# zypher-game/uzkge

Measured on AMD Instinct MI355X. Metric: bn254_g1_msm_points_per_sec, higher is better.
Workload: dtype u256 (254-bit modular integers: 8 x u32 Montgomery limbs in HBM, 9 x 29-bit limbs in the two hot loops); 1 GPU; BN254 G1 MSM, 2^24 random points + uniform scalars per GPU, bases resident in HBM; points_per_gpu=16777216, total_points=16777216

## Files before the change

uzkge_amd/csrc/fp256.hpp:

```cpp
#pragma once
#include <cstdint>

#if defined(__HIPCC__)
#include <hip/hip_runtime.h>
#define UZK_HD __host__ __device__ __forceinline__
#else
#define UZK_HD inline
#endif

namespace uzk {

struct alignas(16) Fp {
    uint32_t v[8];
};

struct FqCfg {
    static constexpr uint32_t M[8] = {0xd87cfd47u, 0x3c208c16u, 0x6871ca8du, 0x97816a91u,
                                      0x8181585du, 0xb85045b6u, 0xe131a029u, 0x30644e72u};
    static constexpr uint32_t R1[8] = {0xc58f0d9du, 0xd35d438du, 0xf5c70b3du, 0x0a78eb28u,
                                       0x7879462cu, 0x666ea36fu, 0x9a07df2fu, 0x0e0a77c1u};
    static constexpr uint32_t R2[8] = {0x538afa89u, 0xf32cfc5bu, 0xd44501fbu, 0xb5e71911u,
                                       0x0a417ff6u, 0x47ab1effu, 0xcab8351fu, 0x06d89f71u};
    static constexpr uint32_t INV = 0xe4866389u;
    static constexpr uint32_t M2[8] = {0xb0f9fa8eu, 0x7841182du, 0xd0e3951au, 0x2f02d522u,
                                       0x0302b0bbu, 0x70a08b6du, 0xc2634053u, 0x60c89ce5u};
};
struct FrCfg {
    static constexpr uint32_t M[8] = {0xf0000001u, 0x43e1f593u, 0x79b97091u, 0x2833e848u,
                                      0x8181585du, 0xb85045b6u, 0xe131a029u, 0x30644e72u};
    static constexpr uint32_t R1[8] = {0x4ffffffbu, 0xac96341cu, 0x9f60cd29u, 0x36fc7695u,
                                       0x7879462eu, 0x666ea36fu, 0x9a07df2fu, 0x0e0a77c1u};
    static constexpr uint32_t R2[8] = {0xae216da7u, 0x1bb8e645u, 0xe35c59e3u, 0x53fe3ab1u,
                                       0x53bb8085u, 0x8c49833du, 0x7f4e44a5u, 0x0216d0b1u};
    static constexpr uint32_t INV = 0xefffffffu;
    static constexpr uint32_t M2[8] = {0xe0000002u, 0x87c3eb27u, 0xf372e122u, 0x5067d090u,
                                       0x0302b0bau, 0x70a08b6du, 0xc2634053u, 0x60c89ce5u};
};

#if defined(__HIP_DEVICE_COMPILE__)
template <class C>
__device__ __forceinline__ Fp mont_mul_fips(const Fp& a, const Fp& b);
template <class C>
__device__ __forceinline__ Fp fp_add_asm(const Fp& a, const Fp& b);
template <class C>
__device__ __forceinline__ Fp fp_sub_asm(const Fp& a, const Fp& b);
template <class C>
__device__ __forceinline__ Fp mont_mul_fips_relaxed(const Fp& a, const Fp& b);
template <class C>
__device__ __forceinline__ Fp fp_add_2m_asm(const Fp& a, const Fp& b);
template <class C>
__device__ __forceinline__ Fp fp_sub_2m_asm(const Fp& a, const Fp& b);
template <class C>
__device__ __forceinline__ void fp_reduce_once_asm(Fp& r);
#endif

template <class C>
struct Field {
    UZK_HD static Fp zero() { Fp r; for (int i = 0; i < 8; ++i) r.v[i] = 0; return r; }
    UZK_HD static Fp one() { Fp r; for (int i = 0; i < 8; ++i) r.v[i] = C::R1[i]; return r; }
    UZK_HD static Fp modulus() { Fp r; for (int i = 0; i < 8; ++i) r.v[i] = C::M[i]; return r; }
    UZK_HD static bool is_zero(const Fp& a) {
        uint32_t o = 0;
        for (int i = 0; i < 8; ++i) o |= a.v[i];
        return o == 0;
    }
    UZK_HD static bool eq(const Fp& a, const Fp& b) {
        uint32_t o = 0;
        for (int i = 0; i < 8; ++i) o |= a.v[i] ^ b.v[i];
        return o == 0;
    }
    UZK_HD static Fp reduce_once(const Fp& a) {
        Fp d; uint64_t br = 0;
        for (int i = 0; i < 8; ++i) {
            uint64_t t = (uint64_t)a.v[i] - C::M[i] - br;
            d.v[i] = (uint32_t)t; br = (t >> 32) & 1;
        }
        Fp r;
        for (int i = 0; i < 8; ++i) r.v[i] = br ? a.v[i] : d.v[i];
        return r;
    }
    UZK_HD static Fp add(const Fp& a, const Fp& b) {
#if defined(__HIP_DEVICE_COMPILE__) && !defined(UZK_PORTABLE_MUL)
        return fp_add_asm<C>(a, b);
#else
        return add_portable(a, b);
#endif
    }
    UZK_HD static Fp add_portable(const Fp& a, const Fp& b) {
        Fp s; uint64_t c = 0;
        for (int i = 0; i < 8; ++i) { c += (uint64_t)a.v[i] + b.v[i]; s.v[i] = (uint32_t)c; c >>= 32; }
        return reduce_once(s);
    }
    UZK_HD static Fp sub(const Fp& a, const Fp& b) {
#if defined(__HIP_DEVICE_COMPILE__) && !defined(UZK_PORTABLE_MUL)
        return fp_sub_asm<C>(a, b);
#else
        return sub_portable(a, b);
#endif
    }
    UZK_HD static Fp sub_portable(const Fp& a, const Fp& b) {
        Fp d; uint64_t br = 0;
        for (int i = 0; i < 8; ++i) {
            uint64_t t = (uint64_t)a.v[i] - b.v[i] - br;
            d.v[i] = (uint32_t)t; br = (t >> 32) & 1;
        }
        uint32_t mask = (uint32_t)0 - (uint32_t)br;
        uint64_t c = 0;
        for (int i = 0; i < 8; ++i) { c += (uint64_t)d.v[i] + (C::M[i] & mask); d.v[i] = (uint32_t)c; c >>= 32; }
        return d;
    }
    UZK_HD static Fp neg(const Fp& a) {
        Fp d; uint64_t br = 0;
        for (int i = 0; i < 8; ++i) {
            uint64_t t = (uint64_t)C::M[i] - a.v[i] - br;
            d.v[i] = (uint32_t)t; br = (t >> 32) & 1;
        }
        bool z = is_zero(a);
        for (int i = 0; i < 8; ++i) d.v[i] = z ? 0u : d.v[i];
        return d;
    }
    UZK_HD static Fp dbl(const Fp& a) { return add(a, a); }

    UZK_HD static Fp mul(const Fp& a, const Fp& b) {
#if defined(__HIP_DEVICE_COMPILE__) && !defined(UZK_PORTABLE_MUL)
        return mont_mul_fips<C>(a, b);
#else
        return mul_portable(a, b);
#endif
    }
    UZK_HD static Fp mul_portable(const Fp& a, const Fp& b) {
#if !defined(__HIP_DEVICE_COMPILE__)
        return mul_host64(a, b);
#else
        return mul_cios32(a, b);
#endif
    }
#if !defined(__HIP_DEVICE_COMPILE__)
    static inline Fp mul_host64(const Fp& a, const Fp& b) {
        typedef unsigned __int128 u128;
        uint64_t x[4], y[4], m[4];
        for (int i = 0; i < 4; ++i) {
            x[i] = (uint64_t)a.v[2 * i] | ((uint64_t)a.v[2 * i + 1] << 32);
            y[i] = (uint64_t)b.v[2 * i] | ((uint64_t)b.v[2 * i + 1] << 32);
            m[i] = (uint64_t)C::M[2 * i] | ((uint64_t)C::M[2 * i + 1] << 32);
        }
        const uint64_t i32 = C::INV;
        const uint64_t inv = i32 * (2 + m[0] * i32);
        uint64_t t[6] = {0, 0, 0, 0, 0, 0};
        for (int i = 0; i < 4; ++i) {
            u128 c = 0;
            for (int j = 0; j < 4; ++j) { c += (u128)x[j] * y[i] + t[j]; t[j] = (uint64_t)c; c >>= 64; }
            c += t[4]; t[4] = (uint64_t)c; t[5] = (uint64_t)(c >> 64);
            const uint64_t q = t[0] * inv;
            c = (u128)q * m[0] + t[0]; c >>= 64;
            for (int j = 1; j < 4; ++j) { c += (u128)q * m[j] + t[j]; t[j - 1] = (uint64_t)c; c >>= 64; }
            c += t[4]; t[3] = (uint64_t)c; t[4] = t[5] + (uint64_t)(c >> 64);
        }
        Fp r;
        for (int i = 0; i < 4; ++i) { r.v[2 * i] = (uint32_t)t[i]; r.v[2 * i + 1] = (uint32_t)(t[i] >> 32); }
        return reduce_once(r);
    }
#endif
    UZK_HD static Fp mul_cios32(const Fp& a, const Fp& b) {
        uint32_t t[9];
        for (int i = 0; i < 9; ++i) t[i] = 0;
#pragma unroll
        for (int i = 0; i < 8; ++i) {
            uint64_t c = 0;
#pragma unroll
            for (int j = 0; j < 8; ++j) {
                c = (uint64_t)a.v[j] * b.v[i] + t[j] + c;
                t[j] = (uint32_t)c; c >>= 32;
            }
            uint32_t t8 = t[8] + (uint32_t)c;
            uint32_t m = t[0] * C::INV;
            c = (uint64_t)m * C::M[0] + t[0];
            c >>= 32;
#pragma unroll
            for (int j = 1; j < 8; ++j) {
                c = (uint64_t)m * C::M[j] + t[j] + c;
                t[j - 1] = (uint32_t)c; c >>= 32;
            }
            c += t8;
            t[7] = (uint32_t)c; t[8] = (uint32_t)(c >> 32);
        }
        Fp r;
        for (int i = 0; i < 8; ++i) r.v[i] = t[i];
        return reduce_once(r);
    }
    UZK_HD static Fp sqr(const Fp& a) { return mul(a, a); }
#if defined(__HIP_DEVICE_COMPILE__)
    __device__ __forceinline__ static Fp mul_rx(const Fp& a, const Fp& b) { return mont_mul_fips_relaxed<C>(a, b); }
    __device__ __forceinline__ static Fp sub_rx(const Fp& a, const Fp& b) { return fp_sub_2m_asm<C>(a, b); }
    __device__ __forceinline__ static Fp add_rx(const Fp& a, const Fp& b) { return fp_add_2m_asm<C>(a, b); }
    __device__ __forceinline__ static Fp dbl_rx(const Fp& a) { return fp_add_2m_asm<C>(a, a); }
    __device__ __forceinline__ static bool is_zero_rx(const Fp& a) {
        uint32_t z = 0, m = 0;
        for (int i = 0; i < 8; ++i) { z |= a.v[i]; m |= a.v[i] ^ C::M[i]; }
        return z == 0 || m == 0;
    }
    __device__ __forceinline__ static Fp canon(const Fp& a) { Fp r = a; fp_reduce_once_asm<C>(r); return r; }
#elif defined(__HIPCC__)
    __device__ static Fp mul_rx(const Fp& a, const Fp& b);
    __device__ static Fp sub_rx(const Fp& a, const Fp& b);
    __device__ static Fp add_rx(const Fp& a, const Fp& b);
    __device__ static Fp dbl_rx(const Fp& a);
    __device__ static bool is_zero_rx(const Fp& a);
    __device__ static Fp canon(const Fp& a);
#endif
    UZK_HD static Fp from_mont(const Fp& a) {
        Fp o = zero(); o.v[0] = 1;
        return mul(a, o);
    }
    UZK_HD static Fp to_mont(const Fp& a) {
        Fp r2; for (int i = 0; i < 8; ++i) r2.v[i] = C::R2[i];
        return mul(a, r2);
    }
};

using Fq = Field<FqCfg>;
using Fr = Field<FrCfg>;

#if defined(__HIP_DEVICE_COMPILE__)
#include "mont_mul_gfx950.inc"
#endif

}
```

uzkge_amd/csrc/msm.hip:

```cpp
#include <algorithm>
#include <cmath>
#include <mutex>
#include <functional>
#include <memory>
#include <condition_variable>
#include <atomic>
#include <cstring>
#include <thread>
#include <vector>

#include "ctx.hpp"
#include "ec29.hpp"
#include "ecquad.hpp"
#include "ecquad29.hpp"
#include "ec29l.hpp"
#include "host_ec64.hpp"
#include "host_math.hpp"

namespace uzk {

constexpr uint32_t kSeg = 16;
constexpr uint32_t kSignBit = 0x80000000u;
constexpr uint32_t kCombineFan = 32;
constexpr int kMaxPasses = 3;

struct MsmWork {
    DevBuf digits, bucket_count, bucket_start, sorted, buckets, partials, win_sums, class_sums, big;
    DevBuf ent[2];
    DevBuf counts[kMaxPasses], segs_start[kMaxPasses], segs_len[kMaxPasses], items[kMaxPasses];
    DevBuf lvl_cnt[2], lvl_off[2], lvl_part[2], small, task_desc, exc;
    XYZZ* h_sums = nullptr;
    size_t h_sums_cap = 0;
    uint32_t* h_max = nullptr;
};

__host__ __device__ inline int msm_num_windows(int c) {
    int W = (254 + c - 1) / c;
    if (254 - (W - 1) * c == c) ++W;
    return W;
}

__device__ __forceinline__ uint32_t msm_fold_scalar_sign(Fp& k) {
    bool gt = false, decided = false;
#pragma unroll
    for (int j = 7; j >= 0; --j) {
        const uint32_t two_k = (k.v[j] << 1) | (j ? (k.v[j - 1] >> 31) : 0u);
        if (!decided && two_k != FrCfg::M[j]) { gt = two_k > FrCfg::M[j]; decided = true; }
    }
    if (!gt) return 0u;
    k = Fr::neg(k);
    return kSignBit;
}


__global__ __launch_bounds__(256) void msm_digits_kernel(ScalarView scalars, uint32_t* __restrict__ digits,
                                                         uint32_t n, uint32_t batch, int c, int W, int w0, int wcnt,
                                                         uint32_t* __restrict__ zero8 = nullptr) {
    const uint64_t t = (uint64_t)blockIdx.x * blockDim.x + threadIdx.x;
    if (zero8 != nullptr && t < 8) zero8[t] = 0;
    if (t >= (uint64_t)n * batch) return;
    const uint32_t b = (uint32_t)(t / n), i = (uint32_t)(t % n);
    Fp k = Fr::from_mont(scalars.at(b, i));
    const uint32_t flip = msm_fold_scalar_sign(k);
    const uint32_t mask = (1u << c) - 1, half = 1u << (c - 1);
    uint32_t carry = 0;
    uint32_t* dst = digits + (size_t)b * wcnt * n + i;
    for (int w = 0; w < w0 + wcnt && w < W; ++w) {
        uint32_t d = (k.v[0] & mask) + carry;
#pragma unroll
        for (int j = 0; j < 7; ++j) k.v[j] = __funnelshift_r(k.v[j], k.v[j + 1], c);
        k.v[7] >>= c;
        uint32_t out;
        if (d > half) { out = ((1u << c) - d) | kSignBit; carry = 1; }
        else { out = d; carry = 0; }
        if (out & ~kSignBit) out ^= flip;
        if (w >= w0) dst[(size_t)(w - w0) * n] = out;
    }
}

__global__ __launch_bounds__(1024) void msm_digits_hist_kernel(ScalarView scalars, uint32_t* __restrict__ digits,
                                                               uint32_t n, int c, int W, uint32_t shift, uint32_t bins,
                                                               uint32_t* __restrict__ counts) {
    extern __shared__ uint32_t hist[];
    const uint32_t ch = blockIdx.x, nch = gridDim.x, b = blockIdx.y;
    const uint32_t cs = (n + nch - 1) / nch;
    const uint32_t lo = min(n, ch * cs), hi = min(n, lo + cs);
    for (uint32_t k = threadIdx.x; k < (uint32_t)W * bins; k += blockDim.x) hist[k] = 0;
    __syncthreads();
    const uint32_t mask = (1u << c) - 1, half = 1u << (c - 1), bmask = bins - 1;
    for (uint32_t i = lo + threadIdx.x; i < hi; i += blockDim.x) {
        Fp k = Fr::from_mont(scalars.at(b, i));
        const uint32_t flip = msm_fold_scalar_sign(k);
        uint32_t carry = 0;
        uint32_t* dst = digits + (size_t)b * W * n + i;
        for (int w = 0; w < W; ++w) {
            uint32_t d = (k.v[0] & mask) + carry;
#pragma unroll
            for (int j = 0; j < 7; ++j) k.v[j] = __funnelshift_r(k.v[j], k.v[j + 1], c);
            k.v[7] >>= c;
            uint32_t out;
            if (d > half) { out = ((1u << c) - d) | kSignBit; carry = 1; }
            else { out = d; carry = 0; }
            if (out & ~kSignBit) out ^= flip;
            dst[(size_t)w * n] = out;
            const uint32_t mag = out & ~kSignBit;
            if (mag) atomicAdd(&hist[(uint32_t)w * bins + (((mag - 1) >> shift) & bmask)], 1u);
        }
    }
    __syncthreads();
    for (uint32_t k = threadIdx.x; k < (uint32_t)W * bins; k += blockDim.x) {
        const uint32_t w = k / bins, bin = k % bins;
        counts[(((size_t)b * W + w) * nch + ch) * bins + bin] = hist[k];
    }
}

struct RadixArgs {
    const uint32_t* digits;
    const uint2* in_entries;
    const uint32_t* seg_start;
    const uint32_t* seg_len;
    uint32_t n;
    uint32_t remap_cnt;
    uint32_t remap_stride, remap_off;
    const uint32_t* item_off;
    uint32_t nseg, chunk;
    uint32_t shift, mask, bins;
    uint32_t* counts;
    uint32_t* prefix;
    uint32_t* bin_base;
    uint32_t* bin_count;
    uint2* out_entries;
    uint32_t* out_vals;
    uint32_t pk_in_bits, pk_out_bits;
    uint32_t seg_min_len;
};
__device__ __forceinline__ uint32_t pk_key(uint32_t e, uint32_t idx_bits) { return e >> (idx_bits + 1); }
__device__ __forceinline__ uint32_t pk_val(uint32_t e, uint32_t idx_bits) {
    return (e & ((1u << idx_bits) - 1)) | (((e >> idx_bits) & 1u) << 31);
}
__device__ __forceinline__ uint32_t pk_make(uint32_t key_low, uint32_t val, uint32_t idx_bits) {
    return (key_low << (idx_bits + 1)) | ((val >> 31) << idx_bits) | (val & ~kSignBit);
}

template <bool FROM_DIGITS>
__device__ __forceinline__ bool radix_work(const RadixArgs& a, uint32_t item, uint32_t& seg, size_t& cidx, uint32_t& base,
                                           uint32_t& lo, uint32_t& hi) {
    if constexpr (FROM_DIGITS) {
        const uint32_t ch = blockIdx.x, nch = gridDim.x;
        seg = blockIdx.y;
        cidx = ((size_t)seg * nch + ch) * a.bins;
        base = 0;
        const uint32_t cs = (a.n + nch - 1) / nch;
        lo = min(a.n, ch * cs);
        hi = min(a.n, lo + cs);
        return true;
    } else {
        if (item >= a.item_off[a.nseg]) return false;
        uint32_t l = 0, h = a.nseg;
        while (h - l > 1) {
            const uint32_t mid = (l + h) >> 1;
            if (a.item_off[mid] <= item) l = mid; else h = mid;
        }
        seg = l;
        cidx = (size_t)item * a.bins;
        base = a.seg_start[seg];
        const uint32_t len = a.seg_len[seg];
        lo = min(len, (item - a.item_off[seg]) * a.chunk);
        hi = min(len, lo + a.chunk);
        return true;
    }
}
template <bool FROM_DIGITS, bool PK_IN>
__device__ __forceinline__ bool radix_load(const RadixArgs& a, uint32_t seg, uint32_t base, uint32_t k, uint32_t& key,
                                           uint32_t& val) {
    if constexpr (FROM_DIGITS) {
        const uint32_t d = a.digits[(size_t)seg * a.n + k];
        const uint32_t mag = d & ~kSignBit;
        key = mag - 1;
        uint32_t idx = k;
        if (a.remap_cnt) idx = (k / a.remap_cnt) * a.remap_stride + a.remap_off + (k % a.remap_cnt);
        val = idx | (d & kSignBit);
        return mag != 0;
    } else if constexpr (PK_IN) {
        const uint32_t e = reinterpret_cast<const uint32_t*>(a.in_entries)[(size_t)base + k];
        key = pk_key(e, a.pk_in_bits);
        val = pk_val(e, a.pk_in_bits);
        return true;
    } else {
        const uint2 e = a.in_entries[(size_t)base + k];
        key = e.x;
        val = e.y;
        return true;
    }
}

template <bool FROM_DIGITS, bool PK_IN>
__global__ __launch_bounds__(1024) void msm_radix_hist_kernel(RadixArgs a) {
    __shared__ uint32_t cnt[512];
    for (uint32_t item = blockIdx.x;; item += gridDim.x) {
        uint32_t seg, base, lo, hi;
        size_t cidx;
        if (!radix_work<FROM_DIGITS>(a, item, seg, cidx, base, lo, hi)) return;
        for (uint32_t b = threadIdx.x; b < a.bins; b += blockDim.x) cnt[b] = 0;
        __syncthreads();
        for (uint32_t k = lo + threadIdx.x; k < hi; k += blockDim.x) {
            if constexpr (FROM_DIGITS) {
                const uint32_t mag = a.digits[(size_t)seg * a.n + k] & ~kSignBit;
                if (mag) atomicAdd(&cnt[((mag - 1) >> a.shift) & a.mask], 1u);
            } else if constexpr (PK_IN) {
                const uint32_t e = reinterpret_cast<const uint32_t*>(a.in_entries)[(size_t)base + k];
                atomicAdd(&cnt[(pk_key(e, a.pk_in_bits) >> a.shift) & a.mask], 1u);
            } else {
                atomicAdd(&cnt[(a.in_entries[(size_t)base + k].x >> a.shift) & a.mask], 1u);
            }
        }
        __syncthreads();
        uint32_t* dst = a.counts + cidx;
        for (uint32_t b = threadIdx.x; b < a.bins; b += blockDim.x) dst[b] = cnt[b];
        if constexpr (FROM_DIGITS) return;
        __syncthreads();
    }
}

__global__ __launch_bounds__(512) void msm_radix_scan_kernel(RadixArgs a, uint32_t nch, const uint32_t* __restrict__ out_start_of,
                                                             uint32_t out_stride) {
    __shared__ uint32_t wsum[8];
    const uint32_t seg = blockIdx.x, b = threadIdx.x, G = gridDim.y, g = blockIdx.y;
    if (a.seg_min_len && a.seg_len[seg] <= a.seg_min_len) return;
    uint32_t run = 0;
    if (b < a.bins) {
        size_t first = (size_t)seg * nch;
        uint32_t cnt = nch;
        if (a.item_off) { first = a.item_off[seg]; cnt = a.item_off[seg + 1] - a.item_off[seg]; }
        const uint32_t per = (cnt + G - 1) / G;
        const uint32_t c0 = min(cnt, g * per), c1 = min(cnt, c0 + per);
        const uint32_t* p0 = a.counts + first * a.bins + b;
        uint32_t r0 = 0, r1 = 0, r2 = 0, r3 = 0;
        uint32_t ch = 0;
        for (; ch + 4 <= c0; ch += 4) {
            r0 += p0[(size_t)ch * a.bins];
            r1 += p0[(size_t)(ch + 1) * a.bins];
            r2 += p0[(size_t)(ch + 2) * a.bins];
            r3 += p0[(size_t)(ch + 3) * a.bins];
        }
        for (; ch < c0; ++ch) r0 += p0[(size_t)ch * a.bins];
        run = r0 + r1 + r2 + r3;
        for (ch = c0; ch < c1; ++ch) {
            const size_t at = (first + ch) * a.bins + b;
            const uint32_t v = a.counts[at];
            a.prefix[at] = run;
            run += v;
        }
    }
    if (g + 1 != G) return;
    uint32_t incl = run;
    for (int o = 1; o < 64; o <<= 1) {
        const uint32_t t = __shfl_up((int)incl, o);
        if ((int)(b & 63) >= o) incl += t;
    }
    if ((b & 63) == 63) wsum[b >> 6] = incl;
    __syncthreads();
    uint32_t pre = 0;
    for (uint32_t w = 0; w < (b >> 6); ++w) pre += wsum[w];
    const uint32_t excl = pre + incl - run;
    if (b < a.bins) {
        const uint32_t start = out_start_of ? out_start_of[seg] : seg * out_stride;
        a.bin_base[(size_t)seg * a.bins + b] = start + excl;
        a.bin_count[(size_t)seg * a.bins + b] = run;
    }
}

__global__ __launch_bounds__(1024) void msm_radix_items_kernel(const uint32_t* __restrict__ seg_len, uint32_t nseg,
                                                               uint32_t chunk, uint32_t* __restrict__ item_off, uint32_t min_len) {
    __shared__ uint32_t part[1024];
    const uint32_t tid = threadIdx.x;
    const uint32_t per = (nseg + 1023) / 1024;
    const uint32_t lo = min(nseg, tid * per), hi = min(nseg, lo + per);
    uint32_t s = 0;
    auto items_of = [&](uint32_t k) { const uint32_t l = seg_len[k]; return l > min_len ? (l + chunk - 1) / chunk : 0u; };
    for (uint32_t k = lo; k < hi; ++k) s += items_of(k);
    part[tid] = s;
    __syncthreads();
    for (uint32_t off = 1; off < 1024; off <<= 1) {
        uint32_t v = (tid >= off) ? part[tid - off] : 0;
        __syncthreads();
        part[tid] += v;
        __syncthreads();
    }
// ... 1432 lines not shown
        g.class_s = 8;
        g.nb2 = std::max<uint32_t>(256, g.NBL >> 8);
    }
    const uint64_t all_entries = (uint64_t)W_total * n * batch;
    const uint64_t mean_pop = (pre ? (uint64_t)W_total * n : (uint64_t)n) >> g.kb;
    g.L = (uint32_t)std::max<uint64_t>(16, std::min<uint64_t>(256, std::min<uint64_t>(4 * mean_pop, all_entries / 200000)));
    g.bound0 = g.entries / g.L + g.TBK;
    g.part_cap = g.bound0 + 2 * g.TBK;
    g.P = g.kb <= 9 ? 1 : (g.kb <= 18 ? 2 : 3);
    g.pk_bits = 0;
    if (g.P == 2 && (!pre || idx_span)) {
        uint32_t ib = 1;
        while ((1ull << ib) < (pre ? idx_span : (uint64_t)g.seg_n)) ++ib;
        const uint32_t first_bits = std::min<uint32_t>(9, g.kb - 1);
        if (ib + 1 + (g.kb - first_bits) <= 32) g.pk_bits = ib;
    }
    uint32_t rem = g.kb, nseg = g.S0;
    for (int p = 0; p < g.P; ++p) {
        uint32_t bits = (rem + (uint32_t)(g.P - p) - 1) / (uint32_t)(g.P - p);
        if (g.pk_bits && p == 0) bits = std::min<uint32_t>(9, g.kb - 1);
        rem -= bits;
        g.sp[p].shift = rem;
        g.sp[p].bins = 1u << bits;
        g.sp[p].nseg = nseg;
        const uint64_t avg = std::max<uint64_t>(1, (g.S0 * (uint64_t)g.seg_n) / nseg);
        g.sp[p].nch = (uint32_t)std::max<uint64_t>(1, std::min<uint64_t>(1024, avg / 32768));
        if (p == 0 && g.pk_bits && avg <= (1ull << 25)) g.sp[p].nch = (uint32_t)((avg + 32767) / 32768);
        g.sp[p].chunk = (p == g.P - 1) ? 16384u : 32768u;
        g.sp[p].items_bound = (uint32_t)(g.entries / g.sp[p].chunk) + nseg;
        nseg *= g.sp[p].bins;
    }
    MsmWork& m = *g.m;
    UZK_TRY(m.digits.reserve((size_t)g.entries * 4));
    UZK_TRY(m.sorted.reserve((size_t)g.entries * 4));
    UZK_TRY(m.bucket_count.reserve((size_t)g.TBK * 4));
    UZK_TRY(m.bucket_start.reserve((size_t)g.TBK * 4));
    UZK_TRY(m.buckets.reserve((size_t)g.TBK * sizeof(XYZZ)));
    UZK_TRY(m.partials.reserve((size_t)2 * g.RW * std::max<uint32_t>(g.groups, g.class_s ? 2 * (g.nb2 / 256 + 1) : 0) * sizeof(XYZZ)));
    UZK_TRY(m.win_sums.reserve((size_t)g.RW * 2 * sizeof(XYZZ)));
    if (g.class_s) UZK_TRY(m.class_sums.reserve((size_t)g.RW * 2 * g.nb2 * sizeof(XYZZ)));
    for (int p = 0; p < g.P; ++p) {
        UZK_TRY(m.counts[p].reserve((size_t)(p == 0 ? 2 * g.sp[p].nseg * g.sp[p].nch : g.sp[p].items_bound) * g.sp[p].bins * 4));
        if (p > 0) UZK_TRY(m.items[p].reserve(((size_t)g.sp[p].nseg + 1) * 4));
        if (p + 1 < g.P) {
            UZK_TRY(m.segs_start[p].reserve((size_t)g.sp[p].nseg * g.sp[p].bins * 4));
            UZK_TRY(m.segs_len[p].reserve((size_t)g.sp[p].nseg * g.sp[p].bins * 4));
            UZK_TRY(m.ent[p & 1].reserve((size_t)g.entries * sizeof(uint2)));
        }
    }
    for (int k = 0; k < 2; ++k) {
        UZK_TRY(m.lvl_cnt[k].reserve((size_t)g.TBK * 4));
        UZK_TRY(m.lvl_off[k].reserve((size_t)g.TBK * 4));
    }
    UZK_TRY(m.lvl_part[0].reserve((size_t)g.part_cap * sizeof(XYZZ)));
    UZK_TRY(m.small.reserve(16384));
    UZK_TRY(m.task_desc.reserve((size_t)g.bound0 * sizeof(TaskDesc)));
    UZK_TRY(m.exc.reserve((size_t)g.bound0 * 4));
    if (m.h_sums_cap < (size_t)g.RW * 2) {
        if (m.h_sums) (void)hipHostFree(m.h_sums);
        UZK_HIP(hipHostMalloc(reinterpret_cast<void**>(&m.h_sums), (size_t)g.RW * 2 * sizeof(XYZZ), hipHostMallocDefault));
        m.h_sums_cap = (size_t)g.RW * 2;
    }
    if (!m.h_max) UZK_HIP(hipHostMalloc(reinterpret_cast<void**>(&m.h_max), 64, hipHostMallocDefault));
    return UZK_OK;
}

static int msm_group_phase1(Ctx& c, MsmGroup& g, const Affine* points, const ScalarView& d_scalars, uint32_t pre_stride,
                            uint32_t pre_off, bool direct_ok = true) {
    MsmWork& m = *g.m;
    hipStream_t st = g.st;
    c.cur_stream = st;
    uint32_t* digits = m.digits.as<uint32_t>();
    uint32_t* sorted = m.sorted.as<uint32_t>();
    uint32_t* bcount = m.bucket_count.as<uint32_t>();
    uint32_t* bstart = m.bucket_start.as<uint32_t>();
    uint32_t* sm = m.small.as<uint32_t>();
    uint32_t* win_tot = sm;
    uint32_t* d_max = sm + 3200;
    UZK_HIP(hipMemsetAsync(d_max, 0, (3912 - 3200) * 4, st));
    const bool fused_hist = !g.pre && g.w0 == 0 && g.W == g.W_total && g.sp[0].nch >= 256 &&
                            (size_t)g.W * g.sp[0].bins * 4 <= 64 * 1024;
    if (fused_hist) {
        KernelScope ks(c, "msm_digits");
        hipLaunchKernelGGL(msm_digits_hist_kernel, dim3(g.sp[0].nch, g.batch), dim3(1024), (size_t)g.W * g.sp[0].bins * 4, st,
                           d_scalars, digits, g.n32, g.cb, (int)g.W, g.sp[0].shift, g.sp[0].bins, m.counts[0].as<uint32_t>());
    } else {
        KernelScope ks(c, "msm_digits");
        const uint64_t tot = (uint64_t)g.n32 * g.batch;
        hipLaunchKernelGGL(msm_digits_kernel, dim3((unsigned)((tot + 255) / 256)), dim3(256), 0, st, d_scalars, digits, g.n32,
                           g.batch, g.cb, (int)g.W_total, (int)g.w0, (int)g.W, (uint32_t*)nullptr);
    }
    for (int p = 0; p < g.P; ++p) {
        const bool first = (p == 0), last = (p == g.P - 1);
        const SortPass& sp = g.sp[p];
        RadixArgs a{};
        a.shift = sp.shift; a.bins = sp.bins; a.mask = sp.bins - 1;
        a.counts = m.counts[p].as<uint32_t>();
        a.prefix = first ? a.counts + (size_t)sp.nseg * sp.nch * sp.bins : a.counts;
        if (first) {
            a.digits = digits;
            a.n = g.seg_n;
            if (g.pre) { a.remap_cnt = g.n32; a.remap_stride = pre_stride; a.remap_off = pre_off; }
        } else {
            a.in_entries = m.ent[(p - 1) & 1].as<uint2>();
            a.seg_start = m.segs_start[p - 1].as<uint32_t>();
            a.seg_len = m.segs_len[p - 1].as<uint32_t>();
        }
        if (g.pk_bits) { if (first) a.pk_out_bits = g.pk_bits; else a.pk_in_bits = g.pk_bits; }
        if (last) { a.bin_base = bstart; a.bin_count = bcount; a.out_vals = sorted; }
        else {
            a.bin_base = m.segs_start[p].as<uint32_t>(); a.bin_count = m.segs_len[p].as<uint32_t>();
            a.out_entries = m.ent[p & 1].as<uint2>();
        }
        int seg_cfg = -1;
        if (last && !first && g.P == 2 && a.pk_in_bits && c.tune_seg_sort && sp.bins <= 512) {
            const double mean = (double)g.seg_n / (double)g.sp[0].bins;
            const double need = mean + 8.0 * std::sqrt(mean) + 64.0;
            for (int k = 0; k < kSegCfgs; ++k)
                if ((double)kSegCap[k] >= need) { seg_cfg = k; break; }
            if (c.tune_seg_sort >= 10) seg_cfg = std::min(kSegCfgs - 1, c.tune_seg_sort - 10);
            if (seg_cfg >= 0) a.seg_min_len = kSegCap[seg_cfg];
        }
        if (!first) {
            a.item_off = m.items[p].as<uint32_t>();
            a.nseg = sp.nseg;
            a.chunk = sp.chunk;
            KernelScope ks(c, "msm_sort_items");
            hipLaunchKernelGGL(msm_radix_items_kernel, dim3(1), dim3(1024), 0, st, a.seg_len, a.nseg, a.chunk,
                               m.items[p].as<uint32_t>(), a.seg_min_len);
        }
        const dim3 grid = first ? dim3(sp.nch, sp.nseg) : dim3(seg_cfg >= 0 ? std::min<uint32_t>(sp.items_bound, 2048u) : sp.items_bound);
        {
            const size_t wgs = first ? 2 * (size_t)grid.x * grid.y : (size_t)sp.items_bound;
            const size_t ent_bytes = g.pk_bits ? 4 : sizeof(uint2);
            const bool ok = m.counts[p].cap >= wgs * sp.bins * 4 &&
                            (last ? (m.bucket_start.cap >= (size_t)sp.nseg * sp.bins * 4 && m.bucket_count.cap >= (size_t)sp.nseg * sp.bins * 4 &&
                                     m.sorted.cap >= (size_t)g.entries * 4)
                                  : (m.segs_start[p].cap >= (size_t)sp.nseg * sp.bins * 4 && m.segs_len[p].cap >= (size_t)sp.nseg * sp.bins * 4 &&
                                     m.ent[p & 1].cap >= (size_t)g.entries * ent_bytes)) &&
                            (first || m.items[p].cap >= ((size_t)sp.nseg + 1) * 4);
            if (!ok) { set_error("msm: sort pass %d: a workspace is smaller than its launch needs (internal error)", p); return UZK_ERR_DEVICE; }
        }
        if (seg_cfg >= 0) {
            KernelScope ks(c, "msm_sort_segment");
            const dim3 sgrid(sp.nseg);
            switch (seg_cfg) {
                case 0: hipLaunchKernelGGL((msm_radix_segment_kernel<128, 12, 1536>), sgrid, dim3(128), 0, st, a); break;
                case 1: hipLaunchKernelGGL((msm_radix_segment_kernel<256, 12, 3072>), sgrid, dim3(256), 0, st, a); break;
                case 2: hipLaunchKernelGGL((msm_radix_segment_kernel<256, 24, 6144>), sgrid, dim3(256), 0, st, a); break;
                case 3: hipLaunchKernelGGL((msm_radix_segment_kernel<256, 40, 10240>), sgrid, dim3(256), 0, st, a); break;
                case 4: hipLaunchKernelGGL((msm_radix_segment_kernel<512, 40, 18432>), sgrid, dim3(512), 0, st, a); break;
                default: hipLaunchKernelGGL((msm_radix_segment_kernel<512, 72, 18432>), sgrid, dim3(512), 0, st, a); break;
            }
        }
        if (!(first && fused_hist)) {
            KernelScope ks(c, "msm_sort_hist");
            if (first) hipLaunchKernelGGL((msm_radix_hist_kernel<true, false>), grid, dim3(1024), 0, st, a);
            else if (a.pk_in_bits) hipLaunchKernelGGL((msm_radix_hist_kernel<false, true>), grid, dim3(256), 0, st, a);
            else hipLaunchKernelGGL((msm_radix_hist_kernel<false, false>), grid, dim3(256), 0, st, a);
        }
        {
            KernelScope ks(c, "msm_sort_scan");
            const uint32_t scan_g = first ? std::max<uint32_t>(1, std::min<uint32_t>(sp.nch / 16, 1024 / std::max<uint32_t>(1, sp.nseg))) : 1u;
            hipLaunchKernelGGL(msm_radix_scan_kernel, dim3(sp.nseg, scan_g), dim3(512), 0, st, a, sp.nch,
                               first ? (const uint32_t*)nullptr : a.seg_start, first ? g.seg_n : 0u);
        }
        {
            KernelScope ks(c, "msm_sort_scatter");
            const uint32_t cs0 = first ? (g.seg_n + sp.nch - 1) / sp.nch : 0u;
            if (first && !last && a.pk_out_bits && sp.bins <= 512 && cs0 <= 32768 && !g.pre)
                hipLaunchKernelGGL((msm_radix_chunk_kernel<512, 64, 18176>), grid, dim3(512), 0, st, a);
            else if (first && last) hipLaunchKernelGGL((msm_radix_scatter_kernel<1024, 8, true, true, false>), grid, dim3(1024), 0, st, a);
            else if (first && g.entries >= (1ull << 26))
                hipLaunchKernelGGL((msm_radix_scatter_kernel<512, 8, true, false, false>), grid, dim3(512), 0, st, a);
            else if (first) hipLaunchKernelGGL((msm_radix_scatter_kernel<1024, 8, true, false, false>), grid, dim3(1024), 0, st, a);
            else if (last && a.pk_in_bits) hipLaunchKernelGGL((msm_radix_scatter_kernel<512, 8, false, true, true>), grid, dim3(512), 0, st, a);
            else if (last) hipLaunchKernelGGL((msm_radix_scatter_kernel<256, 16, false, true, false>), grid, dim3(256), 0, st, a);
            else hipLaunchKernelGGL((msm_radix_scatter_kernel<1024, 8, false, false, false>), grid, dim3(1024), 0, st, a);
        }
    }
    g.cnt_cur = m.lvl_cnt[0].as<uint32_t>();
    g.off_cur = m.lvl_off[0].as<uint32_t>();
    g.base_cur = sm + 1024;
    g.part_cur = m.lvl_part[0].as<XYZZ>();
    uint32_t* len_hist = sm + 3328;
    uint32_t* len_cur = sm + 3328 + kLenBins;
    g.direct = direct_ok;
    XYZZ* direct_buckets = g.direct ? m.buckets.as<XYZZ>() : nullptr;
    {
        KernelScope ks(c, "msm_scan_win");
        hipLaunchKernelGGL(msm_scan_win_kernel, dim3(g.Wd), dim3(1024), scan_win_lds(g.NB), st, bcount, g.L, g.cnt_cur, g.off_cur, win_tot,
                           d_max, g.NB, len_hist);
        hipLaunchKernelGGL(msm_win_base_kernel, dim3(1), dim3(1024), 0, st, win_tot, g.base_cur, g.Wd);
    }
    TaskDesc* desc = m.task_desc.as<TaskDesc>();
    {
        KernelScope ks(c, "msm_task_order");
        uint32_t* big_count = sm + 3908;
        UZK_TRY(m.big.reserve((size_t)(g.TBK + 1) * sizeof(BigBucket)));
        hipLaunchKernelGGL(msm_task_scan_kernel, dim3(1), dim3(256), 0, st, len_hist, len_cur);
        hipLaunchKernelGGL(msm_bucket_fill_kernel, dim3((unsigned)((g.TBK + 255) / 256)), dim3(256), 0, st, g.base_cur, g.cnt_cur, g.off_cur,
                           bstart, bcount, g.NB, g.TBK, len_cur, desc, big_count, m.big.as<BigBucket>(), g.direct ? 1u : 0u);
        hipLaunchKernelGGL(msm_task_fill_big_kernel, dim3(1024), dim3(64), 0, st, big_count, m.big.as<BigBucket>(), len_cur, desc);
    }
    {
        KernelScope ks(c, "msm_accumulate");
        const dim3 grid((unsigned)((g.bound0 + 255) / 256));
        uint32_t* exc_count = sm + 3900;
        uint32_t* exc_list = m.exc.as<uint32_t>();
        hipLaunchKernelGGL(msm_accumulate29_kernel, grid, dim3(256), 0, st, points, sorted, desc, g.base_cur, g.part_cur,
                           g.Wd, exc_count, exc_list, direct_buckets);
        hipLaunchKernelGGL(msm_accumulate_exc_kernel, dim3(std::min<unsigned>(grid.x, 128u)), dim3(256), 0, st, points, sorted, desc, g.part_cur,
                           exc_count, exc_list, direct_buckets);
    }
    UZK_HIP(hipGetLastError());
    UZK_HIP(hipMemcpyAsync(m.h_max, d_max, 4, hipMemcpyDeviceToHost, st));
    return UZK_OK;
}

static int msm_group_phase2(Ctx& c, MsmGroup& g, bool accumulate = false, bool reduce = true) {
    const int a29 = (c.tune_arith29 >> 2) & 1;
    MsmWork& m = *g.m;
    hipStream_t st = g.st;
    c.cur_stream = st;
    UZK_HIP(hipStreamSynchronize(st));
    uint32_t* sm = m.small.as<uint32_t>();
    uint32_t* win_tot = sm;
    uint32_t* win_base[2] = {sm + 1024, sm + 2080};
    XYZZ* buckets = m.buckets.as<XYZZ>();
    XYZZ* partials = m.partials.as<XYZZ>();
    XYZZ* win_sums = m.win_sums.as<XYZZ>();
    const uint32_t G = kCombineFan;
    uint64_t tmax = ((uint64_t)m.h_max[0] + g.L - 1) / g.L;
    const uint32_t gs = g.TBK >= (1u << 18) ? 1u : (tmax > 2 ? 4u : 1u);
    constexpr uint32_t kBigThresh = 4;
    static_assert(sizeof(BigFold) == sizeof(BigBucket), "the two lists share one buffer");
    const bool big_mode = gs == 1 && tmax > kBigThresh;
    uint32_t* big_count = sm + 3904;
    BigFold* big_list = nullptr;
    if (big_mode) {
        UZK_TRY(m.big.reserve((size_t)(g.bound0 / G + g.TBK + 1) * sizeof(BigFold)));
// ... 203 lines not shown
}
bool msm_small_applies(Ctx& c, size_t n, uint32_t batch, int pre_c = 0) {
    if (!c.tune_small || n == 0 || n > (1u << 15)) return false;
    if (pre_c > 10 || (pre_c == 0 && c.msm_window_bits > 10)) return false;
    const int cb = pre_c > 0 ? pre_c : small_window_bits(c, n, batch);
    const uint64_t S = (uint64_t)batch * (uint64_t)msm_num_windows(cb);
    return S <= 65535 && S * n < (1ull << 31);
}

static int msm_run_small(Ctx& c, const Affine* points, const ScalarView& d_scalars, size_t n, uint32_t batch, Jac* out_host, int pre_c,
                         uint32_t pre_stride, uint32_t pre_off) {
    MsmWork& m = c.msm[0];
    hipStream_t st = c.stream;
    c.cur_stream = st;
    const int cb = pre_c > 0 ? pre_c : small_window_bits(c, n, batch);
    const uint32_t W = (uint32_t)msm_num_windows(cb), S = batch * W, NBL = 1u << (cb - 1), n32 = (uint32_t)n;
    const uint64_t entries = (uint64_t)S * n;
    uint32_t L = 0;
    {
        const double lanes = 0.93 * 64.0 * 4.0 * (double)c.num_cus;
        for (int k = 1; k <= 4; ++k) {
            L = (uint32_t)((double)entries / (lanes * k)) + 1;
            if (L <= 12) break;
        }
        L = std::max<uint32_t>(L, 2);
    }
    const uint64_t task_cap = entries / L + (uint64_t)S * NBL;
    SmallLevels lv{};
    uint64_t cap[kSmallMaxLevels + 1];
    cap[0] = task_cap;
    {
        uint64_t worst = (n + L - 1) / L;
        while (worst > 1 && lv.nl < (uint32_t)kSmallMaxLevels) { worst = (worst + kSmallFan - 1) / kSmallFan; ++lv.nl; }
        if (worst > 1) { set_error("msm: small pipeline: %u fold levels do not cover n = %zu at task length %u", lv.nl, n, L); return UZK_ERR_PARAMETER; }
    }
    uint64_t p_total = 0, d_total = 0;
    for (uint32_t k = 0; k <= lv.nl; ++k) {
        if (k > 0) cap[k] = cap[k - 1] / kSmallFan + (uint64_t)S * NBL;
        lv.pbase[k] = (uint32_t)p_total;
        lv.dbase[k] = (uint32_t)d_total;
        p_total += cap[k];
        if (k > 0) d_total += cap[k];
    }
    if (p_total >= (1ull << 32)) { set_error("msm: small pipeline: too many partial sums"); return UZK_ERR_PARAMETER; }
    UZK_TRY(m.digits.reserve((size_t)entries * 4));
    UZK_TRY(m.sorted.reserve((size_t)entries * 4));
    UZK_TRY(m.task_desc.reserve((size_t)task_cap * sizeof(TaskDesc)));
    UZK_TRY(m.lvl_part[0].reserve((size_t)p_total * sizeof(XYZZ)));
    UZK_TRY(m.exc.reserve((size_t)task_cap * 4));
    UZK_TRY(m.partials.reserve((size_t)(d_total + 1) * sizeof(SmallChunk)));
    UZK_TRY(m.bucket_count.reserve((size_t)S * NBL * 4));
    UZK_TRY(m.bucket_start.reserve((size_t)S * kSmallMaxLevels * sizeof(uint2)));
    UZK_TRY(m.win_sums.reserve((size_t)S * sizeof(XYZZ)));
    UZK_TRY(m.small.reserve(16384));
    if (m.h_sums_cap < S) {
        if (m.h_sums) (void)hipHostFree(m.h_sums);
        UZK_HIP(hipHostMalloc(reinterpret_cast<void**>(&m.h_sums), (size_t)S * sizeof(XYZZ), hipHostMallocDefault));
        m.h_sums_cap = S;
    }
    uint32_t* digits = m.digits.as<uint32_t>();
    uint32_t* sorted = m.sorted.as<uint32_t>();
    TaskDesc* desc = m.task_desc.as<TaskDesc>();
    XYZZ* P = m.lvl_part[0].as<XYZZ>();
    SmallChunk* cdesc = m.partials.as<SmallChunk>();
    uint32_t* bucket_ref = m.bucket_count.as<uint32_t>();
    uint2* slot_chunks = m.bucket_start.as<uint2>();
    XYZZ* win_sums = m.h_sums;
    uint32_t* counters = m.small.as<uint32_t>() + 3960;
    const size_t sort_lds = ((size_t)5 * NBL + 32 + n32) * 4;
    {
        static std::once_flag attr_once;
        hipError_t attr_err = hipSuccess;
        std::call_once(attr_once, [&] {
            attr_err = hipFuncSetAttribute(reinterpret_cast<const void*>(msm_small_sort_kernel), hipFuncAttributeMaxDynamicSharedMemorySize,
                                           (5 * 512 + 32 + 32768) * 4);
        });
        UZK_HIP(attr_err);
    }
    {
        HostScope hs(c, "host_msm_enqueue1");
        {
            KernelScope ks(c, "msm_digits");
            const uint64_t tot = (uint64_t)n32 * batch;
            hipLaunchKernelGGL(msm_digits_kernel, dim3((unsigned)((tot + 255) / 256)), dim3(256), 0, st, d_scalars, digits, n32, batch,
                               cb, (int)W, 0, (int)W, counters);
        }
        {
            KernelScope ks(c, "msm_small_sort");
            hipLaunchKernelGGL(msm_small_sort_kernel, dim3(S), dim3(1024), sort_lds, st, digits, n32, NBL, L, sorted, desc, cdesc,
                               bucket_ref, slot_chunks, counters, lv, W, pre_c > 0 ? pre_stride : 0u, pre_off);
        }
        {
            KernelScope ks(c, "msm_accumulate");
            const dim3 grid((unsigned)((task_cap + 255) / 256));
            hipLaunchKernelGGL(msm_accumulate29_kernel, grid, dim3(256), 0, st, points, sorted, desc, counters, P, 0u,
                               counters + 6, m.exc.as<uint32_t>());
            hipLaunchKernelGGL(msm_accumulate_exc_kernel, dim3(256), dim3(256), 0, st, points, sorted, desc, P, counters + 6,
                               m.exc.as<uint32_t>());
        }
        const uint64_t lanes_chip = (uint64_t)c.num_cus * 4 * 64;
        for (uint32_t k = 1; k <= std::min<uint32_t>(lv.nl, 1); ++k) {
            KernelScope ks(c, "msm_small_fold");
            const uint64_t est = k == 1 ? (uint64_t)S * NBL : (uint64_t)S * 2;
            const bool quad = est * 16 <= 10 * lanes_chip;
            const int gs = quad ? 4 : (est * 4 <= 4 * lanes_chip ? 4 : 2);
            const uint64_t lanes = cap[k] * (uint64_t)gs * (quad ? 4 : 1);
            const dim3 grid((unsigned)((lanes + 255) / 256));
            const SmallChunk* cd = cdesc + lv.dbase[k];
#define UZK_FOLD(QD, G) hipLaunchKernelGGL((msm_small_fold_kernel<QD, G>), grid, dim3(256), 0, st, P, cd, counters + k, lv.pbase[k], (c.tune_arith29 >> 2) & 1)
            if (quad) { if (gs >= 8) UZK_FOLD(true, 8); else if (gs >= 4) UZK_FOLD(true, 4); else UZK_FOLD(true, 2); }
            else { if (gs >= 8) UZK_FOLD(false, 8); else if (gs >= 4) UZK_FOLD(false, 4); else if (gs >= 2) UZK_FOLD(false, 2); else UZK_FOLD(false, 1); }
#undef UZK_FOLD
        }
        {
            KernelScope ks(c, "msm_small_reduce");
            const uint32_t Q = std::min<uint32_t>(NBL, 64);
            if ((c.tune_arith29 >> 2) & 1) hipLaunchKernelGGL((msm_small_reduce_kernel<3, 256>), dim3(S), dim3(4 * Q), (size_t)Q * 144, st, P, bucket_ref, cdesc,
                               slot_chunks, lv, win_sums, NBL);
            else hipLaunchKernelGGL((msm_small_reduce_kernel<2, 256>), dim3(S), dim3(4 * Q), (size_t)Q * 144, st, P, bucket_ref, cdesc,
                               slot_chunks, lv, win_sums, NBL);
        }
        UZK_HIP(hipGetLastError());
    }
    {
        HostScope hs(c, "host_msm_wait2");
        UZK_HIP(hipStreamSynchronize(st));
    }
    auto window_sum = [&](uint32_t b, uint32_t w) -> const XYZZ& { return m.h_sums[(size_t)b * W + w]; };
    msm_horner_host(c, batch, W, pre_c > 0 ? 0 : cb, window_sum, out_host);
    return UZK_OK;
}

int msm_run_streamed(Ctx& c, const Affine* points, const Fp* scalars_host, size_t n, Jac* out_host) {
    if (!c.msm) c.msm = new MsmWork[2];
    const int cb = choose_window_bits(n, c.msm_window_bits);
    const uint32_t W = (uint32_t)msm_num_windows(cb);
    std::vector<size_t> bounds{0};
    {
        const size_t cap = (size_t)1 << (c.tune_stream_log > 0 ? std::max(16, std::min(26, c.tune_stream_log)) : 22);
        size_t sz = c.tune_stream_log > 0 ? cap : std::min<size_t>(cap, (size_t)1 << 20);
        int at_this_size = 0;
        while (bounds.back() < n) {
            bounds.push_back(std::min(n, bounds.back() + sz));
            if (++at_this_size >= (sz == ((size_t)1 << 20) ? 2 : 1) && sz < cap) { sz <<= 1; at_this_size = 0; }
        }
    }
    const size_t nchunks = bounds.size() - 1;
    size_t chunk = 0;
    for (size_t k = 0; k < nchunks; ++k) chunk = std::max(chunk, bounds[k + 1] - bounds[k]);
    if (!c.stream2) UZK_HIP(hipStreamCreateWithFlags(&c.stream2, hipStreamNonBlocking));
    hipStream_t copy_st = c.stream2;
    UZK_TRY(c.msm_scalars.reserve(2 * chunk * sizeof(Fp)));
    Fp* stage[2] = {c.msm_scalars.as<Fp>(), c.msm_scalars.as<Fp>() + chunk};
    hipEvent_t up_done[2] = {c.get_event(), c.get_event()}, consumed[2] = {c.get_event(), c.get_event()};
    auto give_back = [&] { for (int i = 0; i < 2; ++i) { c.event_pool.push_back(up_done[i]); c.event_pool.push_back(consumed[i]); } };
    MsmGroup g;
    g.m = &c.msm[0];
    g.st = c.stream;
    int rc = UZK_OK;
    auto upload = [&](size_t k) -> int {
        const size_t lo = bounds[k], len = bounds[k + 1] - lo;
        const int s = (int)(k & 1);
        if (k >= 2) UZK_HIP(hipStreamWaitEvent(copy_st, consumed[s], 0));
        HostScope hs(c, "host_msm_upload");
        UZK_HIP(hipMemcpyAsync(stage[s], scalars_host + lo, len * sizeof(Fp), hipMemcpyHostToDevice, copy_st));
        UZK_HIP(hipEventRecord(up_done[s], copy_st));
        return UZK_OK;
    };
// ... 95 lines not shown
```

Before: 879.6 million points/s.

## Speed up scalar digit recoding and retune radix sort histogram grids

Replaces the from-Montgomery multiply-by-one with a dedicated Montgomery reduction in inline asm. Makes the scalar sign fold branch-free with asm subtract and conditional-select chains. Specialises the digit kernels on a compile-time window size (16/17) so window extraction is fully unrolled. Also unrolls the packed-entry histogram loop by four and caps the later-pass hist and scatter grid sizes at separate limits. These target the digit-extraction and sort-pass overheads, at the cost of more template instantiations and hand-written asm that has to be exactly right.

```diff
diff --git a/uzkge_amd/csrc/fp256.hpp b/uzkge_amd/csrc/fp256.hpp
--- a/uzkge_amd/csrc/fp256.hpp
+++ b/uzkge_amd/csrc/fp256.hpp
@@ -52,6 +52,8 @@
 __device__ __forceinline__ Fp fp_sub_2m_asm(const Fp& a, const Fp& b);
 template <class C>
 __device__ __forceinline__ void fp_reduce_once_asm(Fp& r);
+template <class C>
+__device__ __forceinline__ Fp mont_reduce_fips(const Fp& a);
 #endif
 
 template <class C>
@@ -212,6 +214,31 @@
         Fp o = zero(); o.v[0] = 1;
         return mul(a, o);
     }
+    UZK_HD static Fp from_mont_reduce(const Fp& a) {
+#if defined(__HIP_DEVICE_COMPILE__) && !defined(UZK_PORTABLE_MUL)
+        return mont_reduce_fips<C>(a);
+#else
+        return from_mont_reduce_portable(a);
+#endif
+    }
+    UZK_HD static Fp from_mont_reduce_portable(const Fp& a) {
+        uint32_t t[8];
+        for (int i = 0; i < 8; ++i) t[i] = a.v[i];
+#pragma unroll
+        for (int i = 0; i < 8; ++i) {
+            const uint32_t m = t[0] * C::INV;
+            uint64_t c = ((uint64_t)m * C::M[0] + t[0]) >> 32;
+#pragma unroll
+            for (int j = 1; j < 8; ++j) {
+                c = (uint64_t)m * C::M[j] + t[j] + c;
+                t[j - 1] = (uint32_t)c; c >>= 32;
+            }
+            t[7] = (uint32_t)c;
+        }
+        Fp r;
+        for (int i = 0; i < 8; ++i) r.v[i] = t[i];
+        return reduce_once(r);
+    }
     UZK_HD static Fp to_mont(const Fp& a) {
         Fp r2; for (int i = 0; i < 8; ++i) r2.v[i] = C::R2[i];
         return mul(a, r2);
@@ -223,6 +250,33 @@
 
 #if defined(__HIP_DEVICE_COMPILE__)
 #include "mont_mul_gfx950.inc"
-#endif
-
+
+template <class C>
+__device__ __forceinline__ Fp mont_reduce_fips(const Fp& a) {
+    uint64_t acc = 0;
+    uint32_t top = 0;
+    uint32_t m[8];
+    Fp r;
+    auto mad = [&](uint32_t x, uint32_t y) {
+        asm("v_mad_u64_u32 %0, vcc, %2, %3, %0\n\tv_addc_co_u32_e32 %1, vcc, 0, %1, vcc" : "+v"(acc), "+v"(top) : "v"(x), "s"(y) : "vcc");
+    };
+#pragma unroll
+    for (int k = 0; k < 16; ++k) {
+        if (k < 8) mad(a.v[k], 1u);
+#pragma unroll
+        for (int i = (k < 8 ? 0 : k - 7); i < (k < 8 ? k : 8); ++i) mad(m[i], C::M[k - i]);
+        if (k < 8) {
+            m[k] = (uint32_t)acc * C::INV;
+            mad(m[k], C::M[0]);
+        } else {
+            r.v[k - 8] = (uint32_t)acc;
+        }
+        acc = (acc >> 32) | ((uint64_t)top << 32);
+        top = 0;
+    }
+    fp_reduce_once_asm<C>(r);
+    return r;
 }
+#endif
+
+}
diff --git a/uzkge_amd/csrc/msm.hip b/uzkge_amd/csrc/msm.hip
--- a/uzkge_amd/csrc/msm.hip
+++ b/uzkge_amd/csrc/msm.hip
@@ -34,25 +34,74 @@
     uint32_t* h_max = nullptr;
 };
 
-__host__ __device__ inline int msm_num_windows(int c) {
+__host__ __device__ constexpr int msm_num_windows(int c) {
     int W = (254 + c - 1) / c;
     if (254 - (W - 1) * c == c) ++W;
     return W;
 }
 
+__device__ __forceinline__ constexpr uint32_t msm_half_r(int j) {
+    return (FrCfg::M[j] >> 1) | (j < 7 ? FrCfg::M[j + 1] << 31 : 0u);
+}
 __device__ __forceinline__ uint32_t msm_fold_scalar_sign(Fp& k) {
-    bool gt = false, decided = false;
+    uint32_t n0, n1, n2, n3, n4, n5, n6, n7, tmp, flip;
+    asm("v_sub_co_u32_e32 %0, vcc, %16, %8\n\tv_subb_co_u32_e32 %1, vcc, %17, %9, vcc\n\tv_subb_co_u32_e32 %2, vcc, %18, %10, vcc\n\t"
+        "v_subb_co_u32_e32 %3, vcc, %19, %11, vcc\n\tv_subb_co_u32_e32 %4, vcc, %20, %12, vcc\n\tv_subb_co_u32_e32 %5, vcc, %21, %13, vcc\n\t"
+        "v_subb_co_u32_e32 %6, vcc, %22, %14, vcc\n\tv_subb_co_u32_e32 %7, vcc, %23, %15, vcc"
+        : "=&v"(n0), "=&v"(n1), "=&v"(n2), "=&v"(n3), "=&v"(n4), "=&v"(n5), "=&v"(n6), "=&v"(n7)
+        : "v"(k.v[0]), "v"(k.v[1]), "v"(k.v[2]), "v"(k.v[3]), "v"(k.v[4]), "v"(k.v[5]), "v"(k.v[6]), "v"(k.v[7]),
+          "v"(FrCfg::M[0]), "v"(FrCfg::M[1]), "v"(FrCfg::M[2]), "v"(FrCfg::M[3]), "v"(FrCfg::M[4]), "v"(FrCfg::M[5]), "v"(FrCfg::M[6]), "v"(FrCfg::M[7])
+        : "vcc");
+    asm("v_sub_co_u32_e32 %8, vcc, %18, %0\n\tv_subb_co_u32_e32 %8, vcc, %19, %1, vcc\n\tv_subb_co_u32_e32 %8, vcc, %20, %2, vcc\n\t"
+        "v_subb_co_u32_e32 %8, vcc, %21, %3, vcc\n\tv_subb_co_u32_e32 %8, vcc, %22, %4, vcc\n\tv_subb_co_u32_e32 %8, vcc, %23, %5, vcc\n\t"
+        "v_subb_co_u32_e32 %8, vcc, %24, %6, vcc\n\tv_subb_co_u32_e32 %8, vcc, %25, %7, vcc\n\t"
+        "v_cndmask_b32_e32 %0, %0, %10, vcc\n\tv_cndmask_b32_e32 %1, %1, %11, vcc\n\tv_cndmask_b32_e32 %2, %2, %12, vcc\n\t"
+        "v_cndmask_b32_e32 %3, %3, %13, vcc\n\tv_cndmask_b32_e32 %4, %4, %14, vcc\n\tv_cndmask_b32_e32 %5, %5, %15, vcc\n\t"
+        "v_cndmask_b32_e32 %6, %6, %16, vcc\n\tv_cndmask_b32_e32 %7, %7, %17, vcc\n\tv_cndmask_b32_e64 %9, 0, %26, vcc"
+        : "+v"(k.v[0]), "+v"(k.v[1]), "+v"(k.v[2]), "+v"(k.v[3]), "+v"(k.v[4]), "+v"(k.v[5]), "+v"(k.v[6]), "+v"(k.v[7]), "=&v"(tmp), "=&v"(flip)
+        : "v"(n0), "v"(n1), "v"(n2), "v"(n3), "v"(n4), "v"(n5), "v"(n6), "v"(n7),
+          "v"(msm_half_r(0)), "v"(msm_half_r(1)), "v"(msm_half_r(2)), "v"(msm_half_r(3)), "v"(msm_half_r(4)), "v"(msm_half_r(5)),
+          "v"(msm_half_r(6)), "v"(msm_half_r(7)), "v"(kSignBit)
+        : "vcc");
+    return flip;
+}
+
+template <int C, class Emit>
+__device__ __forceinline__ void msm_recode_scalar(Fp k, uint32_t flip, int c, int wend, Emit&& emit) {
+    uint32_t carry = 0;
+    auto recode = [&](uint32_t raw, uint32_t width_one, uint32_t half) {
+        const uint32_t d = raw + carry;
+        uint32_t out;
+        if (d > half) { out = (width_one - d) | kSignBit; carry = 1; }
+        else { out = d; carry = 0; }
+        if (out & ~kSignBit) out ^= flip;
+        return out;
+    };
+    if constexpr (C > 0) {
+        constexpr int WC = msm_num_windows(C);
 #pragma unroll
-    for (int j = 7; j >= 0; --j) {
-        const uint32_t two_k = (k.v[j] << 1) | (j ? (k.v[j - 1] >> 31) : 0u);
-        if (!decided && two_k != FrCfg::M[j]) { gt = two_k > FrCfg::M[j]; decided = true; }
-    }
-    if (!gt) return 0u;
-    k = Fr::neg(k);
-    return kSignBit;
-}
-
-
+        for (int w = 0; w < WC; ++w) {
+            const int bit = w * C, j = bit >> 5, s = bit & 31;
+            uint32_t raw = 0;
+            if (j < 8) {
+                raw = k.v[j] >> s;
+                if (s + C > 32 && j < 7) raw |= k.v[j + 1] << (32 - s);
+            }
+            if (w < wend) emit(w, recode(raw & ((1u << C) - 1), 1u << C, 1u << (C - 1)));
+        }
+    } else {
+        const uint32_t mask = (1u << c) - 1, half = 1u << (c - 1);
+        for (int w = 0; w < wend; ++w) {
+            const uint32_t raw = k.v[0] & mask;
+#pragma unroll
+            for (int j = 0; j < 7; ++j) k.v[j] = __funnelshift_r(k.v[j], k.v[j + 1], c);
+            k.v[7] >>= c;
+            emit(w, recode(raw, 1u << c, half));
+        }
+    }
+}
+
+template <int C>
 __global__ __launch_bounds__(256) void msm_digits_kernel(ScalarView scalars, uint32_t* __restrict__ digits,
                                                          uint32_t n, uint32_t batch, int c, int W, int w0, int wcnt,
                                                          uint32_t* __restrict__ zero8 = nullptr) {
@@ -60,24 +109,15 @@
     if (zero8 != nullptr && t < 8) zero8[t] = 0;
     if (t >= (uint64_t)n * batch) return;
     const uint32_t b = (uint32_t)(t / n), i = (uint32_t)(t % n);
-    Fp k = Fr::from_mont(scalars.at(b, i));
+    Fp k = Fr::from_mont_reduce(scalars.at(b, i));
     const uint32_t flip = msm_fold_scalar_sign(k);
-    const uint32_t mask = (1u << c) - 1, half = 1u << (c - 1);
-    uint32_t carry = 0;
     uint32_t* dst = digits + (size_t)b * wcnt * n + i;
-    for (int w = 0; w < w0 + wcnt && w < W; ++w) {
-        uint32_t d = (k.v[0] & mask) + carry;
-#pragma unroll
-        for (int j = 0; j < 7; ++j) k.v[j] = __funnelshift_r(k.v[j], k.v[j + 1], c);
-        k.v[7] >>= c;
-        uint32_t out;
-        if (d > half) { out = ((1u << c) - d) | kSignBit; carry = 1; }
-        else { out = d; carry = 0; }
-        if (out & ~kSignBit) out ^= flip;
+    msm_recode_scalar<C>(k, flip, c, min(w0 + wcnt, W), [&](int w, uint32_t out) {
         if (w >= w0) dst[(size_t)(w - w0) * n] = out;
-    }
-}
-
+    });
+}
+
+template <int C>
 __global__ __launch_bounds__(1024) void msm_digits_hist_kernel(ScalarView scalars, uint32_t* __restrict__ digits,
                                                                uint32_t n, int c, int W, uint32_t shift, uint32_t bins,
                                                                uint32_t* __restrict__ counts) {
@@ -87,25 +127,16 @@
     const uint32_t lo = min(n, ch * cs), hi = min(n, lo + cs);
     for (uint32_t k = threadIdx.x; k < (uint32_t)W * bins; k += blockDim.x) hist[k] = 0;
     __syncthreads();
-    const uint32_t mask = (1u << c) - 1, half = 1u << (c - 1), bmask = bins - 1;
+    const uint32_t bmask = bins - 1;
     for (uint32_t i = lo + threadIdx.x; i < hi; i += blockDim.x) {
-        Fp k = Fr::from_mont(scalars.at(b, i));
+        Fp k = Fr::from_mont_reduce(scalars.at(b, i));
         const uint32_t flip = msm_fold_scalar_sign(k);
-        uint32_t carry = 0;
         uint32_t* dst = digits + (size_t)b * W * n + i;
-        for (int w = 0; w < W; ++w) {
-            uint32_t d = (k.v[0] & mask) + carry;
-#pragma unroll
-            for (int j = 0; j < 7; ++j) k.v[j] = __funnelshift_r(k.v[j], k.v[j + 1], c);
-            k.v[7] >>= c;
-            uint32_t out;
-            if (d > half) { out = ((1u << c) - d) | kSignBit; carry = 1; }
-            else { out = d; carry = 0; }
-            if (out & ~kSignBit) out ^= flip;
+        msm_recode_scalar<C>(k, flip, c, C > 0 ? msm_num_windows(C) : W, [&](int w, uint32_t out) {
             dst[(size_t)w * n] = out;
             const uint32_t mag = out & ~kSignBit;
             if (mag) atomicAdd(&hist[(uint32_t)w * bins + (((mag - 1) >> shift) & bmask)], 1u);
-        }
+        });
     }
     __syncthreads();
     for (uint32_t k = threadIdx.x; k < (uint32_t)W * bins; k += blockDim.x) {
@@ -113,6 +144,9 @@
         counts[(((size_t)b * W + w) * nch + ch) * bins + bin] = hist[k];
     }
 }
+
+#define UZK_MSM_DIGITS_DISPATCH(cb, LAUNCH) \
+    do { if ((cb) == 17) { LAUNCH(17); } else if ((cb) == 16) { LAUNCH(16); } else { LAUNCH(0); } } while (0)
 
 struct RadixArgs {
     const uint32_t* digits;
@@ -203,7 +237,19 @@
         if (!radix_work<FROM_DIGITS>(a, item, seg, cidx, base, lo, hi)) return;
         for (uint32_t b = threadIdx.x; b < a.bins; b += blockDim.x) cnt[b] = 0;
         __syncthreads();
-        for (uint32_t k = lo + threadIdx.x; k < hi; k += blockDim.x) {
+        uint32_t k = lo + threadIdx.x;
+        if constexpr (!FROM_DIGITS && PK_IN) {
+            const uint32_t* __restrict__ in = reinterpret_cast<const uint32_t*>(a.in_entries) + base;
+            const uint32_t T = blockDim.x;
+            for (; k + 3 * T < hi; k += 4 * T) {
+                const uint32_t e0 = in[k], e1 = in[k + T], e2 = in[k + 2 * T], e3 = in[k + 3 * T];
+                atomicAdd(&cnt[(pk_key(e0, a.pk_in_bits) >> a.shift) & a.mask], 1u);
+                atomicAdd(&cnt[(pk_key(e1, a.pk_in_bits) >> a.shift) & a.mask], 1u);
+                atomicAdd(&cnt[(pk_key(e2, a.pk_in_bits) >> a.shift) & a.mask], 1u);
+                atomicAdd(&cnt[(pk_key(e3, a.pk_in_bits) >> a.shift) & a.mask], 1u);
+            }
+        }
+        for (; k < hi; k += blockDim.x) {
             if constexpr (FROM_DIGITS) {
                 const uint32_t mag = a.digits[(size_t)seg * a.n + k] & ~kSignBit;
                 if (mag) atomicAdd(&cnt[((mag - 1) >> a.shift) & a.mask], 1u);
@@ -1802,13 +1848,19 @@
                             (size_t)g.W * g.sp[0].bins * 4 <= 64 * 1024;
     if (fused_hist) {
         KernelScope ks(c, "msm_digits");
-        hipLaunchKernelGGL(msm_digits_hist_kernel, dim3(g.sp[0].nch, g.batch), dim3(1024), (size_t)g.W * g.sp[0].bins * 4, st,
-                           d_scalars, digits, g.n32, g.cb, (int)g.W, g.sp[0].shift, g.sp[0].bins, m.counts[0].as<uint32_t>());
+#define UZK_LAUNCH(C) \
+        hipLaunchKernelGGL(msm_digits_hist_kernel<C>, dim3(g.sp[0].nch, g.batch), dim3(1024), (size_t)g.W * g.sp[0].bins * 4, st, \
+                           d_scalars, digits, g.n32, g.cb, (int)g.W, g.sp[0].shift, g.sp[0].bins, m.counts[0].as<uint32_t>())
+        UZK_MSM_DIGITS_DISPATCH(g.cb, UZK_LAUNCH);
+#undef UZK_LAUNCH
     } else {
         KernelScope ks(c, "msm_digits");
         const uint64_t tot = (uint64_t)g.n32 * g.batch;
-        hipLaunchKernelGGL(msm_digits_kernel, dim3((unsigned)((tot + 255) / 256)), dim3(256), 0, st, d_scalars, digits, g.n32,
-                           g.batch, g.cb, (int)g.W_total, (int)g.w0, (int)g.W, (uint32_t*)nullptr);
+#define UZK_LAUNCH(C) \
+        hipLaunchKernelGGL(msm_digits_kernel<C>, dim3((unsigned)((tot + 255) / 256)), dim3(256), 0, st, d_scalars, digits, g.n32, \
+                           g.batch, g.cb, (int)g.W_total, (int)g.w0, (int)g.W, (uint32_t*)nullptr)
+        UZK_MSM_DIGITS_DISPATCH(g.cb, UZK_LAUNCH);
+#undef UZK_LAUNCH
     }
     for (int p = 0; p < g.P; ++p) {
         const bool first = (p == 0), last = (p == g.P - 1);
@@ -1849,7 +1901,9 @@
             hipLaunchKernelGGL(msm_radix_items_kernel, dim3(1), dim3(1024), 0, st, a.seg_len, a.nseg, a.chunk,
                                m.items[p].as<uint32_t>(), a.seg_min_len);
         }
-        const dim3 grid = first ? dim3(sp.nch, sp.nseg) : dim3(seg_cfg >= 0 ? std::min<uint32_t>(sp.items_bound, 2048u) : sp.items_bound);
+        const uint32_t fb_scatter = 768, fb_hist = 512;
+        const dim3 grid = first ? dim3(sp.nch, sp.nseg) : dim3(seg_cfg >= 0 ? std::min<uint32_t>(sp.items_bound, fb_scatter) : sp.items_bound);
+        const dim3 hgrid = (!first && seg_cfg >= 0) ? dim3(std::min<uint32_t>(sp.items_bound, fb_hist)) : grid;
         {
             const size_t wgs = first ? 2 * (size_t)grid.x * grid.y : (size_t)sp.items_bound;
             const size_t ent_bytes = g.pk_bits ? 4 : sizeof(uint2);
@@ -1876,7 +1930,7 @@
         if (!(first && fused_hist)) {
             KernelScope ks(c, "msm_sort_hist");
             if (first) hipLaunchKernelGGL((msm_radix_hist_kernel<true, false>), grid, dim3(1024), 0, st, a);
-            else if (a.pk_in_bits) hipLaunchKernelGGL((msm_radix_hist_kernel<false, true>), grid, dim3(256), 0, st, a);
+            else if (a.pk_in_bits) hipLaunchKernelGGL((msm_radix_hist_kernel<false, true>), hgrid, dim3(256), 0, st, a);
             else hipLaunchKernelGGL((msm_radix_hist_kernel<false, false>), grid, dim3(256), 0, st, a);
         }
         {
@@ -2246,8 +2300,11 @@
         {
             KernelScope ks(c, "msm_digits");
             const uint64_t tot = (uint64_t)n32 * batch;
-            hipLaunchKernelGGL(msm_digits_kernel, dim3((unsigned)((tot + 255) / 256)), dim3(256), 0, st, d_scalars, digits, n32, batch,
-                               cb, (int)W, 0, (int)W, counters);
+#define UZK_LAUNCH(C) \
+            hipLaunchKernelGGL(msm_digits_kernel<C>, dim3((unsigned)((tot + 255) / 256)), dim3(256), 0, st, d_scalars, digits, n32, batch, \
+                               cb, (int)W, 0, (int)W, counters)
+            UZK_MSM_DIGITS_DISPATCH(cb, UZK_LAUNCH);
+#undef UZK_LAUNCH
         }
         {
             KernelScope ks(c, "msm_small_sort");
```

Result: no change. 883.4 million points/s, median of 6 (+0.4%).
